# darnstrom/LinearMPC.jl

Hardware: AMD Instinct MI355X
Metric: condensed-MPC QP solves/sec (batch 1e6 params), pendulum Nc=5 (higher is better)
Workload: dtype f64; 1 GPU; pendulum: inverted pendulum on cart, 4 states / 1 input, Np=50 Nc=5 (n=5 vars, 5 two-sided input bounds, theta=[x;r;u_prev] nth=7), 1000000 parameter points per GPU, cold start, first move u0 returned; batch_per_gpu=1000000, kernel=fast<5>|screen+lane<5>, batches_in_flight=3, rotating_batches=6

## Files before the change

linearmpc.jl_amd/csrc/lmpc_fast_kernel.hpp:

```cpp
#pragma once

#include <hip/hip_runtime.h>
#include <stdint.h>

#include "lmpc_lane_kernel.hpp"
#include "lmpc_tiers.hpp"

namespace lmpc {

#ifndef LMPC_FAST_WAVES
#define LMPC_FAST_WAVES 4
#endif
constexpr int kFastGridWaves = 3;
constexpr int kFastSpinLimit = 1 << 22;
constexpr int kFastTraceSlots = 9;
constexpr int kFastCtrs = 16;
constexpr int kFastMaxTiles = 96;
#ifndef LMPC_FAST_AHEAD
#define LMPC_FAST_AHEAD 1
#endif
constexpr int kFastAhead = LMPC_FAST_AHEAD;

#ifndef LMPC_FAST_DMA_POLICY
#define LMPC_FAST_DMA_POLICY " nt"
#endif
__device__ __forceinline__ void fast_dma16(const void *gsrc, unsigned lds_dst) {
    unsigned keep;
    asm volatile("s_mov_b32 %0, m0\n\ts_mov_b32 m0, %2\n\ts_nop 0\n\tglobal_load_lds_dwordx4 %1, off" LMPC_FAST_DMA_POLICY
                 "\n\ts_mov_b32 m0, %0"
                 : "=&s"(keep) : "v"(gsrc), "s"(lds_dst) : "memory");
}
#ifndef LMPC_FAST_DMA_DEPTH
#define LMPC_FAST_DMA_DEPTH 2
#endif
__host__ __device__ constexpr size_t fast_tile_bytes(int NT) { return (size_t)64 * NT * sizeof(double); }

__device__ __forceinline__ int lds_load(const int *p) {
    return __hip_atomic_load(p, __ATOMIC_RELAXED, __HIP_MEMORY_SCOPE_WORKGROUP);
}

__host__ __device__ constexpr int fast_scr_doubles(int N, int NTHMAX) { return (N * NTHMAX + 2 * N + NTHMAX + 1 + 1) & ~1; }
__host__ __device__ constexpr int fast_const_doubles(int N) { return (N * N + N * (N + 1) / 2 + 2 * N + 1) & ~1; }
__host__ __device__ constexpr int fast_image_doubles(int N, int NTHMAX) { return fast_const_doubles(N) + fast_scr_doubles(N, NTHMAX); }
__host__ __device__ constexpr int fast_image_pieces(int N, int NTHMAX) { return fast_image_doubles(N, NTHMAX) / 2; }
__host__ __device__ constexpr int fast_image_offset(int oFG) { return oFG + kPackFG; }
static_assert(kPackFG % 8 == 0, "the image starts on a 64-byte boundary");
inline bool fast_image_wanted(int N, int n, int m, int ms, int nth) {
    return N >= 2 && N <= 5 && n == N && m == N && ms == N && nth >= 1 && nth <= 16;
}
inline void fast_image_fill(double *buf, const PackLayout &L, int N) {
    const int nconst = N * N + N * (N + 1) / 2 + 2 * N, NTHMAX = L.nthp;
    double *img = buf + fast_image_offset(L.oFG), *scr = img + fast_const_doubles(N);
    for (int i = 0; i < fast_image_doubles(N, NTHMAX); i++) img[i] = 0.0;
    for (int i = 0; i < nconst; i++) img[i] = buf[L.oM + i];
    for (int i = 0; i < N * NTHMAX; i++) scr[i] = buf[L.oDthP + i];
    for (int i = 0; i < 2 * N; i++) scr[N * NTHMAX + i] = buf[L.oBnd + i];
    for (int i = 0; i < NTHMAX; i++) scr[N * NTHMAX + 2 * N + i] = buf[L.oXthP + i];
    scr[N * NTHMAX + 2 * N + NTHMAX] = buf[L.ox0];
}
#ifndef LMPC_FAST_PAY
#define LMPC_FAST_PAY 256
#endif
constexpr int kFastPay = LMPC_FAST_PAY;
__host__ __device__ constexpr size_t fast_lds_bytes(int N, int R, int NTHMAX, bool stage = false) {
    return sizeof(double) * (size_t)(((N * N + N * (N + 1) / 2 + 2 * N + 1) & ~1) + fast_scr_doubles(N, NTHMAX) +
                                     (size_t)kFastPay * (N + (stage ? 0 : 1))) +
           sizeof(int32_t) * ((size_t)R * 64 + 4) + (stage ? (size_t)R * 64 * (sizeof(double) + 1) : 0);
}
__host__ __device__ constexpr size_t fast_lds_bytes_dma(int N, int R, int NTHMAX, int NT, int nstr, int dk, bool stage = false) {
    return fast_lds_bytes(N, R, NTHMAX, stage) + (size_t)dk * nstr * fast_tile_bytes(NT);
}
constexpr size_t kFastCuLds = 160 * 1024;
static_assert(4 * fast_lds_bytes(5, 28, 8, true) <= kFastCuLds, "in-flight shape: four staged workgroups per CU");
static_assert(3 * fast_lds_bytes_dma(5, 21, 8, 7, 3, 2, true) <= kFastCuLds, "stand-alone shape: three staged workgroups per CU");

template <int N> struct FastShifts { double b[N]; };
template <int N> struct FastFallback { double u[N]; unsigned long long act, low; int flag, iter; };
struct FastLoopArgs {
    unsigned long long imm_mask, eq_mask;
    double primal_tol, dual_tol, zero_tol, progress_tol, fval_bound;
    int n, m, words, oM, odu, odl, cycle_tol, iter_limit;
};
__device__ __forceinline__ FastLoopArgs fast_loop_args(const PackLayout &P) {
    return FastLoopArgs{P.imm_mask, P.eq_mask, P.primal_tol, P.dual_tol, P.zero_tol, P.progress_tol, P.fval_bound,
                        P.n, P.m, P.words, P.oM, P.odu, P.odl, P.cycle_tol, P.iter_limit};
}
template <int N>
__device__ __attribute__((noinline)) FastFallback<N> fast_fallback(const FastLoopArgs A, const double *__restrict__ C,
                                                                    const FastShifts<N> sh, const long long pid) {
    PackLayout P{};
    P.imm_mask = A.imm_mask; P.eq_mask = A.eq_mask;
    P.primal_tol = A.primal_tol; P.dual_tol = A.dual_tol; P.zero_tol = A.zero_tol; P.progress_tol = A.progress_tol;
    P.fval_bound = A.fval_bound;
    P.n = A.n; P.m = A.m; P.words = A.words; P.oM = A.oM; P.odu = A.odu; P.odl = A.odl;
    P.cycle_tol = A.cycle_tol; P.iter_limit = A.iter_limit;
    extern __shared__ __align__(16) double lds[];
    const double *sM = lds, *sG = sM + N * N, *sdu = sG + N * (N + 1) / 2, *sdl = sdu + N;
    double sB[N];
#pragma unroll
    for (int j = 0; j < N; j++) sB[j] = sh.b[j];
    LaneState<N, N> s;
    s.init();
    lane_loop<N, N, N, false>(P, C, sM, sG, sdu, sdl, sB, 1, 0, pid, nullptr, s);
    FastFallback<N> r;
#pragma unroll
    for (int c = 0; c < N; c++) r.u[c] = s.u[c];
    r.act = s.act; r.low = s.low; r.flag = s.flag; r.iter = s.iter;
    return r;
}

template <int NTHMAX, int NT, int N, bool GATHER = false, bool STAGE = false>
__device__ __forceinline__ void fast_body(
    const PackLayout &P, const double *__restrict__ C, const double *__restrict__ theta,
    double *__restrict__ X, int32_t *__restrict__ exitflag, int32_t *__restrict__ iters,
    uint64_t *__restrict__ active, long long nprob, int R, int nstr, int32_t *__restrict__ errflag, int spinLimit,
    int dk, int Rs, int Dcap, int32_t *__restrict__ tctr, int32_t *__restrict__ tctr_next) {
    constexpr int KMAX = LMPC_FAST_KMAX < N ? LMPC_FAST_KMAX : N;
    constexpr int nconst = N * N + N * (N + 1) / 2 + 2 * N;
    extern __shared__ __align__(16) double lds[];
    double *sconst = lds;
    double *sScr = sconst + ((nconst + 1) & ~1);
    constexpr bool stage = STAGE;
    constexpr int payw = stage ? N : N + 1;
    double *sPay = sScr + fast_scr_doubles(N, NTHMAX);
    signed char *sF = reinterpret_cast<signed char *>(sPay + (size_t)kFastPay * payw);
    int32_t *ring = reinterpret_cast<int32_t *>(sF + (stage ? R * 64 : 0));
    int *ctrl = reinterpret_cast<int *>(ring + R * 64);
    double *sX = reinterpret_cast<double *>(ctrl + 4);
    char *dma0 = reinterpret_cast<char *>(sX + (stage ? R * 64 : 0));
    const int tid = threadIdx.x, lane = tid & 63;
    const int wv = __builtin_amdgcn_readfirstlane(tid >> 6);
#ifdef LMPC_FAST_TRACE
    const long long trc_entry = (long long)wall_clock64();
#endif
    constexpr bool image = STAGE;
    constexpr int pieces = fast_image_pieces(N, NTHMAX);
    static_assert(fast_image_doubles(N, NTHMAX) % 2 == 0, "the image is a whole number of 16-byte pieces");
    static_assert(fast_const_doubles(N) == ((nconst + 1) & ~1), "image and LDS layout agree");
    static_assert(pieces <= 256, "one piece per thread");
    typedef double img2d __attribute__((ext_vector_type(2)));
    img2d piece = {0.0, 0.0};
    if constexpr (image) {
        if (tid < pieces) piece = reinterpret_cast<const img2d *>(C + fast_image_offset(P.oFG))[tid];
    } else {
        for (int i = tid; i < nconst; i += 256) sconst[i] = C[P.oM + i];
        for (int i = tid; i < N * NTHMAX; i += 256) sScr[i] = C[P.oDthP + i];
        if (tid < 2 * N) sScr[N * NTHMAX + tid] = C[P.oBnd + tid];
        if (tid < NTHMAX) sScr[N * NTHMAX + 2 * N + tid] = C[P.oXthP + tid];
        if (tid == 0) sScr[N * NTHMAX + 2 * N + NTHMAX] = C[P.ox0];
    }
    for (int i = tid; i < R * 64; i += 256) ring[i] = -1;
    if (tid < 4) ctrl[tid] = 0;
    if (image && tid < pieces) reinterpret_cast<img2d *>(lds)[tid] = piece;
    __syncthreads();
    const double *sM = sconst, *sG = sM + N * N, *sdu = sG + N * (N + 1) / 2, *sdl = sdu + N;
    const double ntol = -P.primal_tol;
    const long long ntiles = (nprob + 63) / 64;
#ifdef LMPC_FAST_TRACE
    long long *trc = reinterpret_cast<long long *>(errflag + 16) + ((long long)blockIdx.x * 4 + wv) * kFastTraceSlots;
    int npass = 0;
    if (lane == 0) trc[8] = trc_entry;
#define LMPC_TRC(i) do { if (lane == 0) trc[i] = (long long)wall_clock64(); } while (0)
#else
#define LMPC_TRC(i) do { } while (0)
#endif
    LMPC_TRC(0);
    const bool dyn = tctr != nullptr;
    const long long nstat = dyn ? ((long long)gridDim.x * Rs < ntiles ? (long long)gridDim.x * Rs : ntiles) : ntiles;
    if (dyn && blockIdx.x == 0 && tid < kFastCtrs) tctr_next[tid * 32] = 0;
    const long long t0 = (long long)blockIdx.x * (dyn ? Rs : R);
    const long long t1 = t0 + (dyn ? Rs : R) < nstat ? t0 + (dyn ? Rs : R) : nstat;
    const long long base0 = dyn ? 0 : t0 * 64;

    auto load_record = [&](long long pid, double *dst) {
        const long long pc = pid < nprob ? pid : nprob - 1;
        if constexpr (GATHER) {
            const GatherArgs &Ga = P.gat;
            const int o1 = Ga.nx, o2 = o1 + Ga.nr, o3 = o2 + Ga.nd, o4 = o3 + Ga.nup;
#pragma unroll
            for (int t = 0; t < NT; t++) {
                double v = 0.0;
                if (t < o1) v = Ga.state[pc * Ga.nx + t];
                else if (t < o2) { if (Ga.reference) v = Ga.reference[pc * Ga.nr + (t - o1)]; }
                else if (t < o3) { if (Ga.disturbance) v = Ga.disturbance[pc * Ga.nd + (t - o2)]; }
                else if (t < o4) { if (Ga.control) v = Ga.control[pc * Ga.ncontrol + (t - o3)]; }
                else { if (Ga.parameter) v = Ga.parameter[pc * Ga.np + (t - o4)]; }
                dst[t] = v;
            }
        } else {
            const double *src = theta + pc * NT;
#pragma unroll
            for (int t = 0; t < NT; t++) dst[t] = src[t];
        }
    };
    auto write_x = [&](long long pid, const double (&th)[NT], const double (&u)[N], bool with_u) {
        const double *xk = C + P.oXthP;
        for (int k = 0; k < P.nout; k++, xk += NTHMAX) {
            double sh = C[P.ox0 + k];
#pragma unroll
            for (int t = 0; t < NT; t++) sh = __builtin_fma(xk[t], th[t], sh);
            double xs = 0.0;
            if (with_u) {
#pragma unroll
                for (int c = 0; c < N; c++) xs = __builtin_fma(C[P.oRout + k * N + c], u[c], xs);
            }
            X[pid * P.nout + k] = xs + sh;
        }
    };

    const int role = (wv + (int)(blockIdx.x & 3)) & 3;
    if (role < nstr) {
        double buf[kFastAhead][NT];
        auto process = [&](long long tile, const double (&th)[NT], bool live) {
            const long long pid = tile * 64 + lane;
            const bool valid = live && pid < nprob;
            typedef const double __attribute__((address_space(3))) *lds_cdp;
            unsigned scr_off = (unsigned)(size_t)(lds_cdp)sScr;
            asm volatile("" : "+v"(scr_off));
            const lds_cdp scr = (lds_cdp)(size_t)scr_off;
            bool hard = false;
            typedef double v2d __attribute__((ext_vector_type(2)));
            typedef const v2d __attribute__((address_space(3))) *lds_c2p;
            const lds_c2p c2 = (lds_c2p)(size_t)scr_off;
            static_assert(NTHMAX % 2 == 0, "rows of pairs");
            double bq[N];
#pragma unroll
            for (int j = 0; j < N; j++) {
                double row[NTHMAX];
#pragma unroll
                for (int q = 0; q < (NT + 1) / 2; q++) {
                    const v2d v = c2[j * (NTHMAX / 2) + q];
                    row[2 * q] = v.x; row[2 * q + 1] = v.y;
                }
                double acc = 0.0;
#pragma unroll
                for (int t = 0; t < NT; t++) acc = __builtin_fma(row[t], th[t], acc);
                bq[j] = acc;
                const v2d bb = c2[N * (NTHMAX / 2) + j];
                const double vu = (bb.x + acc) - 0.0;
                const double vl = -((bb.y + acc) - 0.0);
                hard = hard | (vu < ntol) | (vl < ntol);
            }
            hard = hard & valid;
            double sh = scr[N * NTHMAX + 2 * N + NTHMAX];
            {
                double row[NTHMAX];
#pragma unroll
                for (int q = 0; q < (NT + 1) / 2; q++) {
                    const v2d v = c2[(N * NTHMAX + 2 * N) / 2 + q];
                    row[2 * q] = v.x; row[2 * q + 1] = v.y;
                }
#pragma unroll
                for (int t = 0; t < NT; t++) sh = __builtin_fma(row[t], th[t], sh);
            }
            const unsigned long long mask = __ballot(hard);
            if (stage) {
                if (valid) {
                    const int slot = (int)(tile - t0) * 64 + lane;
                    sX[slot] = hard ? sh : 0.0 + sh;
                    sF[slot] = (signed char)(hard ? EXIT_UNFINISHED : EXIT_OPTIMAL);
                }
            } else {
#ifdef LMPC_FAST_NT_STORES
            if (valid) __builtin_nontemporal_store(hard ? EXIT_UNFINISHED : EXIT_OPTIMAL, &exitflag[pid]);
#else
            if (valid) exitflag[pid] = hard ? EXIT_UNFINISHED : EXIT_OPTIMAL;
#endif
            }
            if (mask != 0ull) {
                int base = 0;
                if (lane == 0) base = __hip_atomic_fetch_add(&ctrl[0], __popcll(mask), __ATOMIC_RELAXED, __HIP_MEMORY_SCOPE_WORKGROUP);
                base = __shfl(base, 0);
                if (hard) {
                    const int pos = base + __popcll(mask & ((1ull << lane) - 1ull));
                    if (pos < kFastPay) {
                        double *pay = sPay + pos * payw;
#pragma unroll
                        for (int j = 0; j < N; j++) pay[j] = bq[j];
                        if (!stage) pay[N] = sh;
                    }
                    __hip_atomic_store(&ring[pos], (int32_t)(pid - base0), __ATOMIC_RELEASE, __HIP_MEMORY_SCOPE_WORKGROUP);
                }
            }
            if (!stage && valid && !hard) {
                if (P.nout == 1) {
#ifdef LMPC_FAST_NT_STORES
                    __builtin_nontemporal_store(0.0 + sh, &X[pid]);
#else
                    X[pid] = 0.0 + sh;
#endif
                } else {
                    double u0[N];
#pragma unroll
                    for (int c = 0; c < N; c++) u0[c] = 0.0;
                    write_x(pid, th, u0, false);
                }
                if (iters) iters[pid] = 1;
                if (active) active[pid * P.words] = 0ull;
            }
        };
        if (!GATHER && dk >= 2) {
            constexpr unsigned TB = (unsigned)fast_tile_bytes(NT);
            constexpr int PIECES = (int)((TB + 1023) / 1024);
            constexpr unsigned LASTB = TB - (PIECES - 1) * 1024u;
            typedef const double __attribute__((address_space(3))) *lds_cdp;
            char *dring = dma0 + (size_t)role * dk * TB;
            const unsigned dbase = (unsigned)(size_t)(lds_cdp) reinterpret_cast<double *>(dring);
            const char *tbytes = reinterpret_cast<const char *>(theta);
            const long long tfull = nprob / 64;
            const long long te = t1 < tfull ? t1 : tfull;
            auto issue = [&](long long tile, int slot) {
                const char *src = tbytes + tile * (long long)TB + lane * 16;
#pragma unroll
                for (int p = 0; p < PIECES; p++) {
                    const unsigned dst = __builtin_amdgcn_readfirstlane(dbase + (unsigned)slot * TB + (unsigned)p * 1024u);
                    if (p + 1 < PIECES || LASTB == 1024u || lane * 16 < (int)LASTB) fast_dma16(src + p * 1024, dst);
                }
            };
            int cc = (int)((blockIdx.x * (unsigned)nstr + (unsigned)role) & (kFastCtrs - 1));
            auto take = [&]() -> long long {
                int t = -1;
                if (lane == 0) {
                    if (__hip_atomic_fetch_add(&ctrl[3], 1, __ATOMIC_RELAXED, __HIP_MEMORY_SCOPE_WORKGROUP) < Dcap)
                        t = atomicAdd(&tctr[cc * 32], 1);
                }
                t = __builtin_amdgcn_readfirstlane(t);
                const long long tile = nstat + (long long)t * kFastCtrs + cc;
                return (t >= 0 && tile < ntiles) ? tile : -1;
            };
            if (dk == 2) {
                long long sidx = t0 + role, tk = -1;
                bool drew = false;
                auto take_full = [&]() -> long long { const long long t = take(); return t < tfull ? t : -1; };
                if (dyn && sidx >= te) tk = take_full();
                auto peek = [&]() -> long long { return sidx < te ? sidx : (dyn ? tk : -1); };
                auto advance = [&]() {
                    drew = false;
                    if (sidx < te) { sidx += nstr; if (dyn && sidx >= te) { tk = take_full(); drew = true; } }
                    else if (dyn && tk >= 0) { tk = take_full(); drew = true; }
                };
                long long cur = peek();
                int sc = 0;
                if (cur >= 0) { issue(cur, 0); advance(); }
                while (cur >= 0) {
                    const long long nxt = peek();
                    const bool nd = nxt >= 0;
                    if (nd) { issue(nxt, sc ^ 1); advance(); } else drew = false;
                    if (nd && drew) asm volatile("s_waitcnt vmcnt(%0)" :: "n"(PIECES + 1) : "memory");
                    else if (nd) asm volatile("s_waitcnt vmcnt(%0)" :: "n"(PIECES) : "memory");
                    else asm volatile("s_waitcnt vmcnt(0)" ::: "memory");
                    const double *rec = reinterpret_cast<const double *>(dring + (size_t)sc * TB) + lane * NT;
#pragma unroll
                    for (int t = 0; t < NT; t++) buf[0][t] = rec[t];
                    process(cur, buf[0], true);
                    cur = nxt;
                    sc ^= 1;
                }
                const long long part = dyn ? ((blockIdx.x == 0 && role == 0 && tfull < ntiles) ? tfull : -1)
                                           : ((sidx < t1 && sidx == tfull) ? tfull : -1);
                if (part >= 0) {
                    load_record(part * 64 + lane, buf[0]);
                    process(part, buf[0], true);
                }
            } else {
            const long long first = t0 + role;
            long long ahead = first;
            int sa = 0;
            for (int d = 0; d < dk - 1 && ahead < te; d++, ahead += nstr) { issue(ahead, sa); sa = sa + 1 == dk ? 0 : sa + 1; }
            int sc = 0;
            long long tile = first;
            for (; tile < te; tile += nstr) {
                if (ahead < te) { issue(ahead, sa); sa = sa + 1 == dk ? 0 : sa + 1; ahead += nstr; }
                const long long younger = (ahead - tile) / nstr - 1;
                if (younger >= 2) asm volatile("s_waitcnt vmcnt(%0)" :: "n"(2 * PIECES) : "memory");
                else if (younger == 1) asm volatile("s_waitcnt vmcnt(%0)" :: "n"(PIECES) : "memory");
                else asm volatile("s_waitcnt vmcnt(0)" ::: "memory");
                const double *rec = reinterpret_cast<const double *>(dring + (size_t)sc * TB) + lane * NT;
#pragma unroll
                for (int t = 0; t < NT; t++) buf[0][t] = rec[t];
                sc = sc + 1 == dk ? 0 : sc + 1;
                process(tile, buf[0], true);
            }
            if (tile < t1) {
                load_record(tile * 64 + lane, buf[0]);
                process(tile, buf[0], true);
            }
            if (dyn) {
                long long tl = take();
                while (tl >= 0) {
                    load_record(tl * 64 + lane, buf[0]);
                    const long long nx = take();
                    process(tl, buf[0], true);
                    tl = nx;
                }
            }
            }
        } else
        for (long long base = t0 + role; base < t1; base += (long long)kFastAhead * nstr) {
#pragma unroll
            for (int d = 0; d < kFastAhead; d++) {
                const long long tl = base + (long long)d * nstr;
                load_record((tl < t1 ? tl : base) * 64 + lane, buf[d]);
            }
#pragma unroll
            for (int d = 0; d < kFastAhead; d++) {
                const long long tl = base + (long long)d * nstr;
                process(tl < t1 ? tl : base, buf[d], tl < t1);
            }
        }
        if (dyn && !(!GATHER && dk >= 2)) {
            int cc = (int)((blockIdx.x * (unsigned)nstr + (unsigned)role) & (kFastCtrs - 1));
            auto take = [&]() -> long long {
                int t = -1;
                if (lane == 0) {
                    if (__hip_atomic_fetch_add(&ctrl[3], 1, __ATOMIC_RELAXED, __HIP_MEMORY_SCOPE_WORKGROUP) < Dcap)
                        t = atomicAdd(&tctr[cc * 32], 1);
                }
                t = __builtin_amdgcn_readfirstlane(t);
                const long long tile = nstat + (long long)t * kFastCtrs + cc;
                return (t >= 0 && tile < ntiles) ? tile : -1;
            };
            long long tile = take();
            while (tile >= 0) {
                load_record(tile * 64 + lane, buf[0]);
                const long long nxt = take();
                process(tile, buf[0], true);
                tile = nxt;
            }
        }
        if (lane == 0) __hip_atomic_fetch_add(&ctrl[2], 1, __ATOMIC_RELEASE, __HIP_MEMORY_SCOPE_WORKGROUP);
        LMPC_TRC(1);
    }

    int spins = 0;
    for (;;) {
        int start = 0, n = 0;
        if (lane == 0) {
            for (;;) {
                const int d = __hip_atomic_load(&ctrl[2], __ATOMIC_ACQUIRE, __HIP_MEMORY_SCOPE_WORKGROUP);
                const int w = lds_load(&ctrl[0]);
                int r = lds_load(&ctrl[1]);
                const int avail = w - r;
                if (avail >= 64 || (d >= nstr && avail > 0)) {
                    const int take = avail < 64 ? avail : 64;
                    if (__hip_atomic_compare_exchange_strong(&ctrl[1], &r, r + take, __ATOMIC_RELAXED, __ATOMIC_RELAXED,
                                                             __HIP_MEMORY_SCOPE_WORKGROUP)) { start = r; n = take; break; }
                } else if (d >= nstr) {
                    n = -1;
                    break;
                } else {
                    __builtin_amdgcn_s_sleep(8);
                }
                if (++spins > spinLimit) { n = -2; break; }
            }
        }
        start = __builtin_amdgcn_readfirstlane(start);
        n = __builtin_amdgcn_readfirstlane(n);
        if (n == -2 && lane == 0 && errflag) __hip_atomic_store(errflag, 1, __ATOMIC_RELAXED, __HIP_MEMORY_SCOPE_SYSTEM);
        if (n < 0) break;
#ifdef LMPC_FAST_TRACE
        if (npass < 2) LMPC_TRC(2 + npass);
        npass++;
#endif
#ifdef LMPC_FAST_PRIO
        __builtin_amdgcn_s_setprio(LMPC_FAST_PRIO);
#endif
        const bool mine = lane < n;
        int rel = -1;
        if (mine) {
            int sp = 0;
            while ((rel = __hip_atomic_load(&ring[start + lane], __ATOMIC_ACQUIRE, __HIP_MEMORY_SCOPE_WORKGROUP)) < 0) {
                if (++sp > spinLimit) break;
            }
        }
        if (__any(mine && rel < 0)) {
            if (lane == 0 && errflag) __hip_atomic_store(errflag, 2, __ATOMIC_RELAXED, __HIP_MEMORY_SCOPE_SYSTEM);
            break;
        }
        const long long pid = mine ? base0 + rel : base0;
        double b[N], u[N];
        double sh0 = C[P.ox0];
        const bool handed = start + lane < kFastPay;
#pragma unroll
        for (int j = 0; j < N; j++) b[j] = 0.0;
        if (handed) {
            const double *pay = sPay + (start + (mine ? lane : 0)) * payw;
#pragma unroll
            for (int j = 0; j < N; j++) b[j] = pay[j];
            if (!stage) sh0 = pay[N];
        }
        if (__any(mine && !handed)) {
            double th0[NT];
            load_record(pid, th0);
            const double *dj = C + P.oDthP;
            double sh1 = C[P.ox0];
#pragma unroll
            for (int j = 0; j < N; j++) {
                double acc = 0.0;
#pragma unroll
                for (int t = 0; t < NT; t++) acc = __builtin_fma(dj[j * NTHMAX + t], th0[t], acc);
                b[j] = handed ? b[j] : acc;
            }
            if constexpr (!stage) {
                const double *xk = C + P.oXthP;
#pragma unroll
                for (int t = 0; t < NT; t++) sh1 = __builtin_fma(xk[t], th0[t], sh1);
                sh0 = handed ? sh0 : sh1;
            }
        }
#ifdef LMPC_FAST_TRACE
        if (npass == 1) { if (lane == 0) trc[4] = (long long)(b[0] != 12345.678 ? wall_clock64() : 0); }
#endif
        int iter = 1, nact = 0, wrow[KMAX], flag = EXIT_ITERLIMIT;
        bool wlow[KMAX];
        unsigned long long act = 0ull, low = 0ull;
        const int res = fast_tiers<N, KMAX>(P, sM, sG, sdu, sdl, mine, b, u, iter, wrow, wlow, nact);
        bool solved = res == EXIT_OPTIMAL;
#ifdef LMPC_FAST_TRACE
        if (npass == 1) { if (lane == 0) trc[5] = (long long)(res != 77 ? wall_clock64() : 0); }
#endif
        if (solved) {
            flag = EXIT_OPTIMAL;
#pragma unroll
            for (int i = 0; i < KMAX; i++)
                if (i < nact) { act |= 1ull << wrow[i]; if (wlow[i]) low |= 1ull << wrow[i]; }
        }
#ifndef LMPC_FAST_NO_FALLBACK
        if (mine && !solved) {
            FastShifts<N> bs;
#pragma unroll
            for (int j = 0; j < N; j++) bs.b[j] = b[j];
            const FastFallback<N> r = fast_fallback<N>(fast_loop_args(P), C, bs, pid);
#pragma unroll
            for (int c = 0; c < N; c++) u[c] = r.u[c];
            flag = r.flag; iter = r.iter; act = r.act; low = r.low;
        }
#endif
        if (mine && stage) {
            double xs = 0.0;
#pragma unroll
            for (int c = 0; c < N; c++) xs = __builtin_fma(C[P.oRout + c], u[c], xs);
            const unsigned slot = (unsigned)rel;
            sX[slot] = xs + sX[slot];
            sF[slot] = (signed char)flag;
        } else if (mine) {
            if (P.nout == 1) {
                double xs = 0.0;
#pragma unroll
                for (int c = 0; c < N; c++) xs = __builtin_fma(C[P.oRout + c], u[c], xs);
                X[pid] = xs + sh0;
            } else {
                double th[NT];
                load_record(pid, th);
                write_x(pid, th, u, true);
            }
            exitflag[pid] = flag;
            if (iters) iters[pid] = iter;
            if (active) active[pid * P.words] = (act & ~low) | ((act & low) << N);
        }
#ifdef LMPC_FAST_PRIO
        __builtin_amdgcn_s_setprio(0);
#endif
    }
    if (stage) {
        __syncthreads();
        const long long g0 = t0 * 64;
        const int cnt = (int)((t1 * 64 < nprob ? t1 * 64 : nprob) - g0);
        for (int i = tid; i < cnt; i += 256) __builtin_nontemporal_store(sX[i], &X[g0 + i]);
        for (int i = tid; i < cnt; i += 256) __builtin_nontemporal_store((int32_t)sF[i], &exitflag[g0 + i]);
    }
    LMPC_TRC(6);
#ifdef LMPC_FAST_TRACE
    if (lane == 0) trc[7] = (long long)npass | ((long long)(unsigned)__builtin_amdgcn_s_getreg((31 << 11) | 4) << 16) |
                            ((long long)((unsigned)__builtin_amdgcn_s_getreg((31 << 11) | 20) & 0xffu) << 48);
#endif
#undef LMPC_TRC
}

template <int NTHMAX, int NT, int N, bool GATHER = false>
__global__ __launch_bounds__(256, LMPC_FAST_WAVES) void fast_kernel(
    const PackLayout P, const double *__restrict__ C, const double *__restrict__ theta,
    double *__restrict__ X, int32_t *__restrict__ exitflag, int32_t *__restrict__ iters,
    uint64_t *__restrict__ active, long long nprob, int R, int nstr, int32_t *__restrict__ errflag, int spinLimit,
    int dk, int Rs, int Dcap, int32_t *__restrict__ tctr, int32_t *__restrict__ tctr_next) {
    fast_body<NTHMAX, NT, N, GATHER>(P, C, theta, X, exitflag, iters, active, nprob, R, nstr, errflag, spinLimit, dk, Rs, Dcap, tctr,
                                     tctr_next);
}

template <int NTHMAX, int NT, int N>
__global__ __launch_bounds__(256, LMPC_FAST_WAVES) void fast_staged_kernel(
    const PackLayout P, const double *__restrict__ C, const double *__restrict__ theta,
    double *__restrict__ X, int32_t *__restrict__ exitflag, long long nprob, int R, int nstr, int32_t *__restrict__ errflag,
    int spinLimit, int dk) {
    fast_body<NTHMAX, NT, N, false, true>(P, C, theta, X, exitflag, nullptr, nullptr, nprob, R, nstr, errflag, spinLimit, dk, R, 0,
                                          nullptr, nullptr);
}

constexpr int kFastMaxBatches = 8;
struct FastBatches {
    const double *theta[kFastMaxBatches];
    double *x[kFastMaxBatches];
    int32_t *flag[kFastMaxBatches];
};
template <int NTHMAX, int NT, int N>
__global__ __launch_bounds__(256, LMPC_FAST_WAVES) void fast_kernel_multi(
    const PackLayout P, const double *__restrict__ C, const FastBatches B, long long nprob, int R, int nstr,
    int32_t *__restrict__ errflag, int spinLimit, int dk) {
    const int b = blockIdx.y;
    fast_body<NTHMAX, NT, N, false>(P, C, B.theta[b], B.x[b], B.flag[b], nullptr, nullptr, nprob, R, nstr, errflag, spinLimit, dk, R, 0,
                                    nullptr, nullptr);
}
template <int NTHMAX, int NT, int N>
__global__ __launch_bounds__(256, LMPC_FAST_WAVES) void fast_staged_kernel_multi(
    const PackLayout P, const double *__restrict__ C, const FastBatches B, long long nprob, int R, int nstr,
    int32_t *__restrict__ errflag, int spinLimit, int dk) {
    const int b = blockIdx.y;
    fast_body<NTHMAX, NT, N, false, true>(P, C, B.theta[b], B.x[b], B.flag[b], nullptr, nullptr, nprob, R, nstr, errflag, spinLimit, dk,
                                          R, 0, nullptr, nullptr);
}

}
```

Baseline: 74.77 billion solves/s.

## Split screen/publish and prefetch next tile's theta during publish in staged path

Splits the per-tile work into a screening step and a publishing step. It adds a staged-path loop that issues the next tile's theta loads right after screening, so global loads overlap the publish stores and atomics. The held variant preloads the first few constant rows from LDS and pins registers to force that ordering. In the staged path the ring store becomes relaxed after an explicit lgkmcnt wait, and the shuffle of the ring base becomes readfirstlane. These add register pressure and rely on hand-written wait ordering being correct.

```diff
diff --git a/linearmpc.jl_amd/csrc/lmpc_fast_kernel.hpp b/linearmpc.jl_amd/csrc/lmpc_fast_kernel.hpp
--- a/linearmpc.jl_amd/csrc/lmpc_fast_kernel.hpp
+++ b/linearmpc.jl_amd/csrc/lmpc_fast_kernel.hpp
@@ -2,6 +2,8 @@
 
 #include <hip/hip_runtime.h>
 #include <stdint.h>
+
+#include <type_traits>
 
 #include "lmpc_lane_kernel.hpp"
 #include "lmpc_tiers.hpp"
@@ -20,6 +22,12 @@
 #define LMPC_FAST_AHEAD 1
 #endif
 constexpr int kFastAhead = LMPC_FAST_AHEAD;
+#ifndef LMPC_FAST_TURN
+#define LMPC_FAST_TURN 1
+#endif
+#ifndef LMPC_FAST_TURN_EARLY
+#define LMPC_FAST_TURN_EARLY 1
+#endif
 
 #ifndef LMPC_FAST_DMA_POLICY
 #define LMPC_FAST_DMA_POLICY " nt"
@@ -34,6 +42,12 @@
 #define LMPC_FAST_DMA_DEPTH 2
 #endif
 __host__ __device__ constexpr size_t fast_tile_bytes(int NT) { return (size_t)64 * NT * sizeof(double); }
+
+__device__ __forceinline__ void fast_pin(double &s) { asm volatile("" : "+v"(s) :: "memory"); }
+template <int N> __device__ __forceinline__ void fast_pin(double (&b)[N]) {
+#pragma unroll
+    for (int j = 0; j < N; j++) fast_pin(b[j]);
+}
 
 __device__ __forceinline__ int lds_load(const int *p) {
     return __hip_atomic_load(p, __ATOMIC_RELAXED, __HIP_MEMORY_SCOPE_WORKGROUP);
@@ -211,9 +225,8 @@
     const int role = (wv + (int)(blockIdx.x & 3)) & 3;
     if (role < nstr) {
         double buf[kFastAhead][NT];
-        auto process = [&](long long tile, const double (&th)[NT], bool live) {
-            const long long pid = tile * 64 + lane;
-            const bool valid = live && pid < nprob;
+        auto screen = [&](auto held, double (&th)[NT], const bool valid, double (&bq)[N], double &shift) -> bool {
+            constexpr bool HELD = decltype(held)::value;
             typedef const double __attribute__((address_space(3))) *lds_cdp;
             unsigned scr_off = (unsigned)(size_t)(lds_cdp)sScr;
             asm volatile("" : "+v"(scr_off));
@@ -223,13 +236,23 @@
             typedef const v2d __attribute__((address_space(3))) *lds_c2p;
             const lds_c2p c2 = (lds_c2p)(size_t)scr_off;
             static_assert(NTHMAX % 2 == 0, "rows of pairs");
-            double bq[N];
+            constexpr int RQ = (NT + 1) / 2, NA = !HELD ? 0 : (NT > 8 ? 1 : (20 / RQ < N ? 20 / RQ : N));
+            v2d ahead[NA ? NA : 1][RQ];
+            if constexpr (HELD) {
+#pragma unroll
+                for (int j = 0; j < NA; j++)
+#pragma unroll
+                    for (int q = 0; q < RQ; q++) ahead[j][q] = c2[j * (NTHMAX / 2) + q];
+                fast_pin(th);
+            }
 #pragma unroll
             for (int j = 0; j < N; j++) {
                 double row[NTHMAX];
 #pragma unroll
                 for (int q = 0; q < (NT + 1) / 2; q++) {
-                    const v2d v = c2[j * (NTHMAX / 2) + q];
+                    v2d v;
+                    if (j < NA) v = ahead[j][q];
+                    else v = c2[j * (NTHMAX / 2) + q];
                     row[2 * q] = v.x; row[2 * q + 1] = v.y;
                 }
                 double acc = 0.0;
@@ -253,6 +276,12 @@
 #pragma unroll
                 for (int t = 0; t < NT; t++) sh = __builtin_fma(row[t], th[t], sh);
             }
+            shift = sh;
+            return hard;
+        };
+        auto publish = [&](long long tile, const double (&bq)[N], const double sh, const bool hard, const bool valid,
+                           const double (&th)[NT]) {
+            const long long pid = tile * 64 + lane;
             const unsigned long long mask = __ballot(hard);
             if (stage) {
                 if (valid) {
@@ -270,7 +299,8 @@
             if (mask != 0ull) {
                 int base = 0;
                 if (lane == 0) base = __hip_atomic_fetch_add(&ctrl[0], __popcll(mask), __ATOMIC_RELAXED, __HIP_MEMORY_SCOPE_WORKGROUP);
-                base = __shfl(base, 0);
+                if constexpr (stage) base = __builtin_amdgcn_readfirstlane(base);
+                else base = __shfl(base, 0);
                 if (hard) {
                     const int pos = base + __popcll(mask & ((1ull << lane) - 1ull));
                     if (pos < kFastPay) {
@@ -279,7 +309,12 @@
                         for (int j = 0; j < N; j++) pay[j] = bq[j];
                         if (!stage) pay[N] = sh;
                     }
-                    __hip_atomic_store(&ring[pos], (int32_t)(pid - base0), __ATOMIC_RELEASE, __HIP_MEMORY_SCOPE_WORKGROUP);
+                    if constexpr (stage) {
+                        asm volatile("s_waitcnt lgkmcnt(0)" ::: "memory");
+                        __hip_atomic_store(&ring[pos], (int32_t)(pid - base0), __ATOMIC_RELAXED, __HIP_MEMORY_SCOPE_WORKGROUP);
+                    } else {
+                        __hip_atomic_store(&ring[pos], (int32_t)(pid - base0), __ATOMIC_RELEASE, __HIP_MEMORY_SCOPE_WORKGROUP);
+                    }
                 }
             }
             if (!stage && valid && !hard) {
@@ -298,6 +333,12 @@
                 if (iters) iters[pid] = 1;
                 if (active) active[pid * P.words] = 0ull;
             }
+        };
+        auto process = [&](long long tile, double (&th)[NT], bool live) {
+            const bool valid = live && tile * 64 + lane < nprob;
+            double bq[N], sh;
+            const bool hard = screen(std::false_type{}, th, valid, bq, sh);
+            publish(tile, bq, sh, hard, valid, th);
         };
         if (!GATHER && dk >= 2) {
             constexpr unsigned TB = (unsigned)fast_tile_bytes(NT);
@@ -395,6 +436,39 @@
                 }
             }
             }
+        } else if constexpr (STAGE && LMPC_FAST_TURN) {
+            const long long first = t0 + role;
+            if (first < t1) {
+                const uintptr_t last = reinterpret_cast<uintptr_t>(theta + (nprob - 1) * NT);
+                const uintptr_t step = (uintptr_t)nstr * (64 * NT * sizeof(double));
+                uintptr_t at = reinterpret_cast<uintptr_t>(theta + (first * 64 + lane) * NT);
+                typedef const double __attribute__((address_space(1))) *glb_cdp;
+                auto request = [&]() {
+                    const glb_cdp src = (glb_cdp)(at < last ? at : last);
+#pragma unroll
+                    for (int t = 0; t < NT; t++) buf[0][t] = src[t];
+                };
+                request();
+                for (long long tile = first;; tile += nstr) {
+                    const bool more = tile + nstr < t1;
+#ifdef LMPC_FAST_TURN_PRIO
+                    __builtin_amdgcn_s_setprio(LMPC_FAST_TURN_PRIO);
+#endif
+                    double bq[N], sh;
+                    const bool valid = tile * 64 + lane < nprob;
+                    const bool hard = screen(std::true_type{}, buf[0], valid, bq, sh);
+                    fast_pin(bq);
+                    fast_pin(sh);
+                    at += step;
+                    if (LMPC_FAST_TURN_EARLY && more) request();
+#ifdef LMPC_FAST_TURN_PRIO
+                    __builtin_amdgcn_s_setprio(0);
+#endif
+                    publish(tile, bq, sh, hard, valid, buf[0]);
+                    if (!more) break;
+                    if (!LMPC_FAST_TURN_EARLY) request();
+                }
+            }
         } else
         for (long long base = t0 + role; base < t1; base += (long long)kFastAhead * nstr) {
 #pragma unroll
```

Measured after the change: 76.44 billion solves/s (median of 6 runs). +2.2%, better.
